# ManuelWendl/Monocular_Visual_Odometry_VA4MR

Hardware: AMD Instinct MI355X
Metric: frames/s + ATE vs ref, KITTI seq00 1241x376 @ 1/2/4/8 MI355X (higher is better)
Workload: dtype mixed(u8,i32,f32,f64)

## Files before the change

monocular_visual_odometry_va4mr_amd/csrc/vo_pyr.hip:

```cpp
#include "vo_dev.h"

namespace {


#define PT_W 128
#define PT_H 16
#ifndef PYR0_TH
#define PYR0_TH 32
#endif
#define PV_W (PT_W + 8)
#define PV_H (PT_H + 2)
#define PS_H (2 * PV_H + 3)
#define PS_W ((2 * PV_W + 3 + 8 + 3) / 4 * 4)

struct PyrLevelArgs {
    const uint8_t* src;
    int64_t sstride;
    int sw, sh, spitch;
    int64_t soff;
    uint8_t* pyr;
    int64_t pstride;
    int16_t* der;
    int64_t dstride;
    int w, h, pitch;
    int64_t off;
    int level;
};

template <bool L0, int TH, bool FSRC>
VO_DEV void pyr_tile(const PyrLevelArgs& A, int px0, int py0)
{
    constexpr int PH = TH + 2, SH = 2 * PH + 3, RPT = TH / 8;
    __shared__ uint32_t PVw[PH * PV_W / 4];
    __shared__ int yk[PH], xc[PV_W];
    __shared__ int mm[4];
    uint8_t* PV = (uint8_t*)PVw;
    const int tid = threadIdx.x;
    const int b = blockIdx.z;
    const int pw = A.w + 2 * VO_BORDER, ph = A.h + 2 * VO_BORDER;
    if (tid < 4) mm[tid] = (tid & 1) ? -1 : 0x7fffffff;
    __syncthreads();
    if (tid < PH) {
        const int py = py0 - 1 + tid;
        const int y = (py >= 0 && py < ph) ? refl101(py - VO_BORDER, A.h) : -1;
        yk[tid] = y;
        if (y >= 0) { atomicMin(&mm[0], y); atomicMax(&mm[1], y); }
    }
    if (tid < PV_W) {
        const int px = px0 - 4 + tid;
        const int x = (px >= 0 && px < pw) ? refl101(px - VO_BORDER, A.w) : -1;
        xc[tid] = x;
        if (x >= 0) { atomicMin(&mm[2], x); atomicMax(&mm[3], x); }
    }
    __syncthreads();
    constexpr int NPV = (PH * PV_W + 255) / 256;
    if constexpr (L0) {
        const uint8_t* fr = A.src + (int64_t)b * A.sstride;
        uint32_t v[NPV];
#pragma unroll
        for (int i = 0; i < NPV; ++i) {
            const int e = tid + 256 * i;
            const int ee = min(e, PH * PV_W - 1);
            const int k = ee / PV_W, c = ee - k * PV_W;
            const int y = yk[k], x = xc[c];
            v[i] = fr[(int64_t)max(y, 0) * A.w + max(x, 0)];
            if (y < 0 || x < 0) v[i] = 0;
        }
#pragma unroll
        for (int i = 0; i < NPV; ++i) {
            const int e = tid + 256 * i;
            if (e < PH * PV_W) PV[e] = (uint8_t)v[i];
        }
    } else {
        __shared__ uint32_t SRw[SH * PS_W / 4];
        __shared__ uint2 HSw[SH * PV_W / 4];
        const uint8_t* SR = (const uint8_t*)SRw;
        const int sy0 = 2 * mm[0] - 2, sy1 = 2 * mm[1] + 2;
        const int sx0 = 2 * mm[2] - 2, sx1 = 2 * mm[3] + 2;
        const int nsr = sy1 - sy0 + 1;
        const int gx0 = sx0 + VO_BORDER;
        const int ax0 = gx0 & ~3, sh = gx0 - ax0;
        const int nwd = (sx1 + VO_BORDER - ax0) / 4 + 1;
        constexpr int NSR = (SH * (PS_W / 4) + 255) / 256;
        uint32_t v[NSR];
        if constexpr (FSRC) {
            const uint8_t* fr = A.src + (int64_t)b * A.sstride;
#pragma unroll
            for (int i = 0; i < NSR; ++i) {
                const int e = tid + 256 * i;
                const int r = e / (PS_W / 4), c = e - r * (PS_W / 4);
                const bool in = r < nsr && c < nwd;
                const uint8_t* row = fr + (int64_t)refl101(sy0 + (in ? r : 0), A.sh) * A.sw;
                const int cb = ax0 - VO_BORDER + 4 * (in ? c : 0);
                v[i] = (uint32_t)row[refl101(cb, A.sw)] | ((uint32_t)row[refl101(cb + 1, A.sw)] << 8) |
                       ((uint32_t)row[refl101(cb + 2, A.sw)] << 16) | ((uint32_t)row[refl101(cb + 3, A.sw)] << 24);
            }
        } else {
            const uint8_t* sbase = A.src + (int64_t)b * A.sstride + A.soff + ax0;
#pragma unroll
            for (int i = 0; i < NSR; ++i) {
                const int e = tid + 256 * i;
                const int r = e / (PS_W / 4), c = e - r * (PS_W / 4);
                const bool in = r < nsr && c < nwd;
                v[i] = *(const uint32_t*)(sbase + (int64_t)(sy0 + (in ? r : 0) + VO_BORDER) * A.spitch + 4 * (in ? c : 0));
            }
        }
#pragma unroll
        for (int i = 0; i < NSR; ++i) {
            const int e = tid + 256 * i;
            if (e < SH * (PS_W / 4)) SRw[e] = v[i];
        }
        __syncthreads();
        static_assert(PV_W % 4 == 0, "pyrDown column quads");
        constexpr int PQ = PV_W / 4;
        uint2* HS2 = HSw;
        for (int e = tid; e < nsr * PQ; e += 256) {
            const int r = e / PQ, cq = e - r * PQ;
            const int x0 = xc[4 * cq], x3 = xc[4 * cq + 3];
            uint32_t o[4];
            if (x0 >= 0 && x3 == x0 + 3 && xc[4 * cq + 1] == x0 + 1 && xc[4 * cq + 2] == x0 + 2) {
                const int ob = r * PS_W + sh + (2 * x0 - 2 - sx0);
                const uint32_t* wp = SRw + (ob >> 2);
                const uint32_t sa = (uint32_t)(ob & 3);
                const uint32_t W0 = wp[0], W1 = wp[1], W2 = wp[2], W3 = wp[3];
                const uint32_t T0 = __builtin_amdgcn_alignbyte(W1, W0, sa);
                const uint32_t T1 = __builtin_amdgcn_alignbyte(W2, W1, sa);
                const uint32_t T2 = __builtin_amdgcn_alignbyte(W3, W2, sa);
                constexpr uint32_t K4 = 0x04060401u;
                o[0] = __builtin_amdgcn_udot4(T0, K4, T1 & 0xffu, false);
                o[1] = __builtin_amdgcn_udot4(__builtin_amdgcn_alignbyte(T1, T0, 2), K4, (T1 >> 16) & 0xffu, false);
                o[2] = __builtin_amdgcn_udot4(T1, K4, T2 & 0xffu, false);
                o[3] = __builtin_amdgcn_udot4(__builtin_amdgcn_alignbyte(T2, T1, 2), K4, (T2 >> 16) & 0xffu, false);
            } else {
#pragma unroll
                for (int i = 0; i < 4; ++i) {
                    const int x = xc[4 * cq + i];
                    o[i] = 0;
                    if (x >= 0) {
                        const uint8_t* q = SR + r * PS_W + sh + (2 * x - 2 - sx0);
                        o[i] = q[0] + 4 * q[1] + 6 * q[2] + 4 * q[3] + q[4];
                    }
                }
            }
            HS2[r * PQ + cq] = make_uint2(o[0] | (o[1] << 16), o[2] | (o[3] << 16));
        }
        __syncthreads();
        const uint2* HSq = HSw;
        for (int e = tid; e < PH * PQ; e += 256) {
            const int k = e / PQ, cq = e - k * PQ;
            const int y = yk[k];
            uint32_t v = 0;
            if (y >= 0) {
                const uint2* q = HSq + (2 * y - 2 - sy0) * PQ + cq;
                const uint2 q0 = q[0], q1 = q[PQ], q2 = q[2 * PQ], q3 = q[3 * PQ], q4 = q[4 * PQ];
                const uint32_t ax = q0.x + 4 * q1.x + 6 * q2.x + 4 * q3.x + q4.x + 0x00800080u;
                const uint32_t ay = q0.y + 4 * q1.y + 6 * q2.y + 4 * q3.y + q4.y + 0x00800080u;
                v = __builtin_amdgcn_perm(ay, ax, 0x07050301u);
            }
            PVw[k * (PV_W / 4) + cq] = v;
        }
    }    __syncthreads();
    const int tc = tid & 31, tr = tid >> 5;
    const int px = px0 + 4 * tc;
#pragma unroll
    for (int rr = 0; rr < RPT; ++rr) {
        const int k = 1 + RPT * tr + rr;
        const int py = py0 + RPT * tr + rr;
        if (py >= ph || px >= A.pitch) continue;
        const uint32_t* rowc = PVw + (k * PV_W) / 4 + 1 + tc;
        *(uint32_t*)(A.pyr + (int64_t)b * A.pstride + A.off + (int64_t)py * A.pitch + px) = rowc[0];
        const int y = py - VO_BORDER, x0 = px - VO_BORDER;
        if (!A.der || y < 0 || y >= A.h || x0 + 3 < 0 || x0 >= A.w) continue;
        uint32_t o[4];
        const uint32_t* ru = rowc - PV_W / 4;
        const uint32_t* rl = rowc + PV_W / 4;
        const uint64_t U = ((uint64_t)ru[0] << 8) | (ru[-1] >> 24), L = ((uint64_t)rl[0] << 8) | (rl[-1] >> 24),
                       Cc = ((uint64_t)rowc[0] << 8) | (rowc[-1] >> 24);
        const uint64_t U5 = U | ((uint64_t)(ru[1] & 0xff) << 40), L5 = L | ((uint64_t)(rl[1] & 0xff) << 40),
                       C5 = Cc | ((uint64_t)(rowc[1] & 0xff) << 40);
#pragma unroll
        for (int i = 0; i < 4; ++i) {
            int dx = 0, dy = 0;
            const int x = x0 + i;
            if (x >= 0 && x < A.w) {
                const int ul = (int)((U5 >> (8 * i)) & 0xff), uc = (int)((U5 >> (8 * i + 8)) & 0xff),
                          ur = (int)((U5 >> (8 * i + 16)) & 0xff);
                const int ll = (int)((L5 >> (8 * i)) & 0xff), lc = (int)((L5 >> (8 * i + 8)) & 0xff),
                          lr = (int)((L5 >> (8 * i + 16)) & 0xff);
                const int cl = (int)((C5 >> (8 * i)) & 0xff), cr = (int)((C5 >> (8 * i + 16)) & 0xff);
                const int t0l = (ul + ll) * 3 + cl * 10;
                const int t0r = (ur + lr) * 3 + cr * 10;
                dx = t0r - t0l;
                dy = ((lr - ur) + (ll - ul)) * 3 + (lc - uc) * 10;
            }
            o[i] = (uint32_t)(uint16_t)(int16_t)dx | ((uint32_t)(uint16_t)(int16_t)dy << 16);
        }
        int16_t* dq = A.der + (int64_t)b * A.dstride + 2 * (A.off + (int64_t)py * A.pitch + px);
        *(uint4*)dq = make_uint4(o[0], o[1], o[2], o[3]);
    }
}


__global__ void __launch_bounds__(256) k_pyr01(PyrLevelArgs A0, PyrLevelArgs A1, int tx0, int ty0, int tx1)
{
    if ((int)blockIdx.y < ty0) {
        if ((int)blockIdx.x < tx0) pyr_tile<true, PYR0_TH, false>(A0, blockIdx.x * PT_W, blockIdx.y * PYR0_TH);
    } else if ((int)blockIdx.x < tx1) {
        pyr_tile<false, PT_H, true>(A1, blockIdx.x * PT_W, (blockIdx.y - ty0) * PT_H);
    }
}

#define PR_STEP 248
template <bool L0, bool RAGGED = false>
VO_DEV void pyr_rows_wave(const PyrLevelArgs& A, int R, int sx, int sy, int b)
{
    const int lane = lane_id();
    const int wo = A.w, ho = A.h;
    const int pw = wo + 2 * VO_BORDER, ph = ho + 2 * VO_BORDER;
    const int pwa = (pw + 3) & ~3;
    const int ns = (pwa + PR_STEP - 1) / PR_STEP;
    const bool lastst = sx == ns - 1;
    const int base = lastst ? max(pwa - 252, -4) : sx * PR_STEP - 4;
    const int px = base + 4 * lane;
    const int y0 = sy * R;
    if (y0 >= ho || sx >= ns) return;
    const int y1 = min(y0 + R, ho);
    const int lo = lastst ? max(pwa - PR_STEP, 0) : sx * PR_STEP;
    const int hi = lastst ? pwa : min(sx * PR_STEP + PR_STEP, pwa - PR_STEP);
    const bool wlane = lane >= 1 && lane <= 62 && px >= lo && px < hi && px < pw;
    const bool dlane = wlane && px + 3 >= VO_BORDER && px < VO_BORDER + wo;
    int fsrc[4];
#pragma unroll
    for (int j = 0; j < 4; ++j) {
        const int c = px + j;
        const int sp = (c >= 0 && c < pw) ? VO_BORDER + refl101(c - VO_BORDER, wo) : c;
        const int rel = sp - base;
        fsrc[j] = (rel >= 0 && rel < 256) ? rel : 4 * lane + j;
    }
    const bool fixcols = base < VO_BORDER || base + 256 > VO_BORDER + wo;
    auto fix = [&](uint32_t v) -> uint32_t {
        if (!fixcols) return v;
        uint32_t o = 0;
#pragma unroll
        for (int j = 0; j < 4; ++j) {
            const uint32_t t = (uint32_t)__builtin_amdgcn_ds_bpermute((fsrc[j] >> 2) << 2, (int)v);
            o |= ((t >> (8 * (fsrc[j] & 3))) & 0xffu) << (8 * j);
        }
        return o;
    };
    const __amdgpu_buffer_rsrc_t rs =
        __builtin_amdgcn_make_buffer_rsrc((void*)(A.src + (int64_t)b * A.sstride), (short)0, (int)A.sstride, 0x00020000);
    uint8_t* dst = A.pyr + (int64_t)b * A.pstride + A.off;
    auto put_row = [&](int y, uint32_t v) {
        if (!wlane) return;
        *(uint32_t*)(dst + (int64_t)(VO_BORDER + y) * A.pitch + px) = v;
        if (ho >= VO_BORDER + 2) {
            if (y >= 1 && y <= VO_BORDER) *(uint32_t*)(dst + (int64_t)(VO_BORDER - y) * A.pitch + px) = v;
            if (y >= ho - 1 - VO_BORDER && y <= ho - 2)
                *(uint32_t*)(dst + (int64_t)(VO_BORDER + 2 * ho - 2 - y) * A.pitch + px) = v;
        } else {
            for (int py = 0; py < ph; ++py) {
                if (py == VO_BORDER) py = VO_BORDER + ho;
                if (py < ph && refl101(py - VO_BORDER, ho) == y) *(uint32_t*)(dst + (int64_t)py * A.pitch + px) = v;
            }
        }
    };
    auto put_der = [&](int y, uint32_t u, uint32_t c, uint32_t l) {
        const uint32_t ul = (uint32_t)__builtin_amdgcn_update_dpp(0, (int)u, 0x138, 0xF, 0xF, false);
        const uint32_t cl = (uint32_t)__builtin_amdgcn_update_dpp(0, (int)c, 0x138, 0xF, 0xF, false);
        const uint32_t ll = (uint32_t)__builtin_amdgcn_update_dpp(0, (int)l, 0x138, 0xF, 0xF, false);
        const uint32_t ur = (uint32_t)__builtin_amdgcn_update_dpp(0, (int)u, 0x130, 0xF, 0xF, false);
        const uint32_t cr = (uint32_t)__builtin_amdgcn_update_dpp(0, (int)c, 0x130, 0xF, 0xF, false);
        const uint32_t lr = (uint32_t)__builtin_amdgcn_update_dpp(0, (int)l, 0x130, 0xF, 0xF, false);
        if (!dlane || !A.der) return;
        const uint64_t U5 = ((uint64_t)u << 8) | (ul >> 24) | ((uint64_t)(ur & 0xff) << 40);
        const uint64_t L5 = ((uint64_t)l << 8) | (ll >> 24) | ((uint64_t)(lr & 0xff) << 40);
        const uint64_t C5 = ((uint64_t)c << 8) | (cl >> 24) | ((uint64_t)(cr & 0xff) << 40);
        uint32_t o[4];
#pragma unroll
        for (int i = 0; i < 4; ++i) {
            int dx = 0, dy = 0;
            const int x = px + i - VO_BORDER;
            if (x >= 0 && x < wo) {
                const int uL = (int)((U5 >> (8 * i)) & 0xff), uc = (int)((U5 >> (8 * i + 8)) & 0xff),
                          uR = (int)((U5 >> (8 * i + 16)) & 0xff);
                const int lL = (int)((L5 >> (8 * i)) & 0xff), lc = (int)((L5 >> (8 * i + 8)) & 0xff),
                          lR = (int)((L5 >> (8 * i + 16)) & 0xff);
                const int cL = (int)((C5 >> (8 * i)) & 0xff), cR = (int)((C5 >> (8 * i + 16)) & 0xff);
                dx = ((uR + lR) * 3 + cR * 10) - ((uL + lL) * 3 + cL * 10);
                dy = ((lR - uR) + (lL - uL)) * 3 + (lc - uc) * 10;
            }
            o[i] = (uint32_t)(uint16_t)(int16_t)dx | ((uint32_t)(uint16_t)(int16_t)dy << 16);
        }
        int16_t* dq = A.der + (int64_t)b * A.dstride + 2 * (A.off + (int64_t)(VO_BORDER + y) * A.pitch + px);
        *(uint4*)dq = make_uint4(o[0], o[1], o[2], o[3]);
    };
    if constexpr (L0) {
        auto ld_dw = [&](int o) -> uint32_t {
            uint32_t v = __builtin_amdgcn_raw_buffer_load_b32(rs, o, 0, 0);
            if constexpr (RAGGED) {
                const int fbytes = (int)A.sstride;
                if (o < fbytes && o + 4 > fbytes) {
                    v = 0;
#pragma unroll
                    for (int k = 0; k < 3; ++k) v |= (uint32_t)(uint8_t)__builtin_amdgcn_raw_buffer_load_b8(rs, o + k, 0, 0) << (8 * k);
                }
            }
            return v;
        };
        auto ld_row = [&](int y, uint32_t& d0, uint32_t& d1) {
            const int ro = y * wo + base - VO_BORDER;
            const int al = (ro & ~3) + 4 * lane;
            d0 = ld_dw(al);
            d1 = ld_dw(al + 4);
        };
        auto val = [&](int y, uint32_t d0, uint32_t d1) {
            return fix(__builtin_amdgcn_alignbyte(d1, d0, (uint32_t)((y * wo + base - VO_BORDER) & 3)));
        };
        uint32_t a0, a1, c0, c1, n0, n1;
        const int yh = refl101(y0 - 1, ho);
        ld_row(yh, a0, a1);
        ld_row(y0, c0, c1);
        ld_row(y0 + 1 < y1 ? y0 + 1 : refl101(y1, ho), n0, n1);
        uint32_t vu = val(yh, a0, a1);
        uint32_t vc = val(y0, c0, c1);
        put_row(y0, vc);
        for (int y = y0; y < y1; ++y) {
            const int yn = y + 1 < y1 ? y + 1 : refl101(y1, ho);
            const uint32_t vl = val(yn, n0, n1);
            const int y2 = y + 2 < y1 ? y + 2 : refl101(y1, ho);
            if (y + 1 < y1) ld_row(y2, n0, n1);
            if (y + 1 < y1) put_row(y + 1, vl);
            put_der(y, vu, vc, vl);
            vu = vc;
            vc = vl;
        }
    } else {
        const int loff = 2 * px - VO_BORDER;
        auto ld_src = [&](int sr, uint32_t& d0, uint32_t& d1) {
            const int o = (int)A.soff + (VO_BORDER + sr) * A.spitch + loff;
            d0 = __builtin_amdgcn_raw_buffer_load_b32(rs, o, 0, 0);
            d1 = __builtin_amdgcn_raw_buffer_load_b32(rs, o + 4, 0, 0);
        };
        constexpr uint32_t K4 = 0x04060401u;
        auto hsum = [&](uint32_t D0, uint32_t D1, uint32_t& h01, uint32_t& h23) {
            const uint32_t L1 = (uint32_t)__builtin_amdgcn_update_dpp(0, (int)D1, 0x138, 0xF, 0xF, false);
            const uint32_t R0 = (uint32_t)__builtin_amdgcn_update_dpp(0, (int)D0, 0x130, 0xF, 0xF, false);
            const uint32_t o0 = __builtin_amdgcn_udot4(__builtin_amdgcn_alignbyte(D0, L1, 2), K4, (D0 >> 16) & 0xffu, false);
            const uint32_t o1 = __builtin_amdgcn_udot4(D0, K4, D1 & 0xffu, false);
            const uint32_t o2 = __builtin_amdgcn_udot4(__builtin_amdgcn_alignbyte(D1, D0, 2), K4, (D1 >> 16) & 0xffu, false);
            const uint32_t o3 = __builtin_amdgcn_udot4(D1, K4, R0 & 0xffu, false);
            h01 = o0 | (o1 << 16);
            h23 = o2 | (o3 << 16);
        };
        auto vert = [&](const uint32_t (&hx)[5], const uint32_t (&hy)[5]) {
            const uint32_t ax = hx[0] + 4 * hx[1] + 6 * hx[2] + 4 * hx[3] + hx[4] + 0x00800080u;
            const uint32_t ay = hy[0] + 4 * hy[1] + 6 * hy[2] + 4 * hy[3] + hy[4] + 0x00800080u;
            return fix(__builtin_amdgcn_perm(ay, ax, 0x07050301u));
        };
        auto direct = [&](int y) {
            uint32_t d[5][2], hx[5], hy[5];
#pragma unroll
            for (int k = 0; k < 5; ++k) ld_src(2 * y - 2 + k, d[k][0], d[k][1]);
#pragma unroll
            for (int k = 0; k < 5; ++k) hsum(d[k][0], d[k][1], hx[k], hy[k]);
            return vert(hx, hy);
        };
        uint32_t hx[5], hy[5];
        {
            uint32_t d[5][2];
#pragma unroll
            for (int k = 0; k < 5; ++k) ld_src(2 * y0 - 2 + k, d[k][0], d[k][1]);
#pragma unroll
            for (int k = 0; k < 5; ++k) hsum(d[k][0], d[k][1], hx[k], hy[k]);
        }
        uint32_t p0, p1, q0, q1;
        ld_src(2 * y0 + 3, p0, p1);
        ld_src(2 * y0 + 4, q0, q1);
        uint32_t vu = direct(refl101(y0 - 1, ho));
        uint32_t vc = vert(hx, hy);
        put_row(y0, vc);
        for (int y = y0; y < y1; ++y) {
            uint32_t vl;
            if (y + 1 < y1) {
                hx[0] = hx[2]; hy[0] = hy[2];
                hx[1] = hx[3]; hy[1] = hy[3];
                hx[2] = hx[4]; hy[2] = hy[4];
                hsum(p0, p1, hx[3], hy[3]);
                hsum(q0, q1, hx[4], hy[4]);
                ld_src(2 * y + 5, p0, p1);
                ld_src(2 * y + 6, q0, q1);
                vl = vert(hx, hy);
                put_row(y + 1, vl);
            } else {
                vl = direct(refl101(y1, ho));
            }
            put_der(y, vu, vc, vl);
            vu = vc;
            vc = vl;
        }
    }
}

template <bool L0, bool RAGGED = false>
__global__ void __launch_bounds__(64) k_pyr_rows(PyrLevelArgs A, int R)
{
    pyr_rows_wave<L0, RAGGED>(A, R, (int)blockIdx.x, (int)blockIdx.y, (int)blockIdx.z);
}

#define PYR_TAIL_MAX 6
struct PyrTailArgs {
    PyrLevelArgs a[PYR_TAIL_MAX];
    int R[PYR_TAIL_MAX];
    int n;
};
__global__ void __launch_bounds__(1024) k_pyr_tail(PyrTailArgs T)
{
    const int w = wave_id(), nw = (int)(blockDim.x >> 6);
    for (int l = 0; l < T.n; ++l) {
        const PyrLevelArgs& A = T.a[l];
        const int R = T.R[l];
        const int pwa = (A.w + 2 * VO_BORDER + 3) & ~3;
        const int ns = (pwa + PR_STEP - 1) / PR_STEP, nch = (A.h + R - 1) / R;
        for (int it = w; it < ns * nch; it += nw) pyr_rows_wave<false>(A, R, it % ns, it / ns, (int)blockIdx.x);
        __syncthreads();
    }
}

__global__ void __launch_bounds__(256) k_scharr(const uint8_t* __restrict__ pyr, int64_t pstride,
                                                int16_t* __restrict__ der, int64_t dstride,
                                                int w, int h, int pitch, int64_t off)
{
    const int b = blockIdx.z;
    const int px0 = (blockIdx.x * 64 + lane_id()) * 4;
    const int py = blockIdx.y * 4 + wave_id();
    if (px0 >= w + 2 * VO_BORDER || py >= h + 2 * VO_BORDER) return;
    const int y = py - VO_BORDER;
    const uint8_t* c = pyr + b * pstride + off + (int64_t)py * pitch;
    const uint8_t* u = c - pitch;
    const uint8_t* l = c + pitch;
    uint32_t o[4];
#pragma unroll
    for (int k = 0; k < 4; ++k) {
        const int px = px0 + k, x = px - VO_BORDER;
        int dx = 0, dy = 0;
        if (x >= 0 && x < w && y >= 0 && y < h) {
            const int t0l = (u[px - 1] + l[px - 1]) * 3 + c[px - 1] * 10;
            const int t0r = (u[px + 1] + l[px + 1]) * 3 + c[px + 1] * 10;
            const int t1l = l[px - 1] - u[px - 1], t1c = l[px] - u[px], t1r = l[px + 1] - u[px + 1];
            dx = t0r - t0l;
            dy = (t1r + t1l) * 3 + t1c * 10;
        }
        o[k] = (uint32_t)(uint16_t)(int16_t)dx | ((uint32_t)(uint16_t)(int16_t)dy << 16);
    }
    int16_t* dq = der + b * dstride + 2 * (off + (int64_t)py * pitch + px0);
    *(uint4*)dq = make_uint4(o[0], o[1], o[2], o[3]);
}

}

static bool pyr_level_args(const vo_dims* d, const vo_state* s, int cur, int l, const uint8_t* frames,
                           int64_t frame_stride, PyrLevelArgs* A)
{
    if (l == 0) {
        A->src = frames; A->sstride = frame_stride; A->sw = A->sh = A->spitch = 0; A->soff = 0;
    } else {
        A->src = s->pyr[cur]; A->sstride = d->pyr_stride;
        A->sw = d->lvl_w[l - 1]; A->sh = d->lvl_h[l - 1]; A->spitch = d->lvl_pitch[l - 1]; A->soff = d->lvl_off[l - 1];
    }
    A->pyr = s->pyr[cur]; A->pstride = d->pyr_stride;
    A->der = s->der[cur]; A->dstride = d->der_stride;
    A->w = d->lvl_w[l]; A->h = d->lvl_h[l]; A->pitch = d->lvl_pitch[l]; A->off = d->lvl_off[l];
    A->level = l;
    return A->pitch % 64 == 0 && A->pitch >= A->w + 2 * VO_BORDER;
}

extern "C" int vo_pyr_build(const vo_dims* d, const vo_state* s, int cur, const uint8_t* frames,
                            int64_t frame_stride, vo_stream_t stream)
{
    if (!d || !s || !frames || cur < 0 || cur > 1 || d->nlev < 1) return VO_EARG;
    static const int p01_env = vo_env_int("VO_PYR01", -1);
    const bool fuse01 = d->nlev >= 2 && (p01_env >= 0 ? p01_env == 1 : d->B <= 8);
    if (fuse01) {
        PyrLevelArgs A0, A1;
        if (!pyr_level_args(d, s, cur, 0, frames, frame_stride, &A0)) return VO_EARG;
        if (!pyr_level_args(d, s, cur, 1, frames, frame_stride, &A1)) return VO_EARG;
        A1.src = frames; A1.sstride = frame_stride; A1.spitch = 0; A1.soff = 0;
        const int pw0 = A0.w + 2 * VO_BORDER, ph0 = A0.h + 2 * VO_BORDER;
        const int pw1 = A1.w + 2 * VO_BORDER, ph1 = A1.h + 2 * VO_BORDER;
        const int tx0 = (pw0 + PT_W - 1) / PT_W, ty0 = (ph0 + PYR0_TH - 1) / PYR0_TH;
        const int tx1 = (pw1 + PT_W - 1) / PT_W, ty1 = (ph1 + PT_H - 1) / PT_H;
        dim3 g(tx0 > tx1 ? tx0 : tx1, ty0 + ty1, d->B);
        hipLaunchKernelGGL(k_pyr01, g, dim3(256), 0, VO_STREAM(stream), A0, A1, tx0, ty0, tx1);
    }
    static const int tail_env = vo_env_int("VO_PYR_TAIL", -1);
    const int ltail = 2;
    const bool tail = d->nlev > ltail && d->nlev - ltail <= PYR_TAIL_MAX &&
                      (tail_env >= 0 ? tail_env == 1 : d->B > 8 && d->B <= 64);
    PyrTailArgs T;
    T.n = tail ? d->nlev - ltail : 0;
    for (int i = 0; i < T.n; ++i) {
        PyrLevelArgs& A = T.a[i];
        if (!pyr_level_args(d, s, cur, ltail + i, frames, frame_stride, &A)) return VO_EARG;
        const int pwa = (A.w + 2 * VO_BORDER + 3) & ~3, ns = (pwa + PR_STEP - 1) / PR_STEP;
        const int want = ns >= 16 ? 1 : 16 / ns;
        const int R = (A.h + want - 1) / want;
        T.R[i] = R < 2 ? 2 : R;
    }
    const int lend = tail ? ltail : d->nlev;
    for (int l = fuse01 ? 2 : 0; l < lend; ++l) {
        PyrLevelArgs A;
        if (!pyr_level_args(d, s, cur, l, frames, frame_stride, &A)) return VO_EARG;
        const int pw = A.w + 2 * VO_BORDER;
        const int ns = ((pw + 3) / 4 * 4 + PR_STEP - 1) / PR_STEP;
        int R = 16;
        while (R > 4 && (int64_t)ns * ((A.h + R - 1) / R) * d->B < 8192) R >>= 1;
        dim3 g(ns, (A.h + R - 1) / R, d->B);
        if (l == 0 && (frame_stride & 3)) hipLaunchKernelGGL((k_pyr_rows<true, true>), g, dim3(64), 0, VO_STREAM(stream), A, R);
        else if (l == 0) hipLaunchKernelGGL(k_pyr_rows<true>, g, dim3(64), 0, VO_STREAM(stream), A, R);
        else hipLaunchKernelGGL(k_pyr_rows<false>, g, dim3(64), 0, VO_STREAM(stream), A, R);
    }
    if (tail) hipLaunchKernelGGL(k_pyr_tail, dim3(d->B), dim3(1024), 0, VO_STREAM(stream), T);
    return hip_ok() ? VO_OK : VO_EHIP;
}

extern "C" int vo_pyr_deriv(const vo_dims* d, const vo_state* s, int which, vo_stream_t stream)
{
    if (!d || !s || which < 0 || which > 1) return VO_EARG;
    for (int l = 0; l < d->nlev; ++l) {
        const int pw = d->lvl_w[l] + 2 * VO_BORDER, ph = d->lvl_h[l] + 2 * VO_BORDER;
        dim3 g((pw + 4 * 64 - 1) / (4 * 64), (ph + 3) / 4, d->B);
        hipLaunchKernelGGL(k_scharr, g, dim3(256), 0, VO_STREAM(stream), s->pyr[which], d->pyr_stride, s->der[which],
                           d->der_stride, d->lvl_w[l], d->lvl_h[l], d->lvl_pitch[l], d->lvl_off[l]);
    }
    return hip_ok() ? VO_OK : VO_EHIP;
}
```

Before: 86860.

## Vectorize pyramid Scharr derivative with packed 16-bit math and buffer stores

Rewrites the per-row derivative computation in the pyramid row kernel to use packed 16-bit vector arithmetic on unpacked byte pairs, with DPP lane shifts and alignbyte instead of per-pixel 64-bit shifting. Adds a specialized inner-row loop, split on whether column fixup is needed, that removes reflection branches and uses incremental offsets. Stores go through buffer resources, L1+ levels load with 64-bit buffer loads, and a waves-per-EU occupancy hint plus a readfirstlane are added. Together these cut ALU and branch overhead in the pyramid/derivative stage. The cost is more code paths and a border-masking scheme that must keep matching the previous output.

Result: no change. 87650 (median of 6 runs) (+0.9%).

```diff
diff --git a/monocular_visual_odometry_va4mr_amd/csrc/vo_pyr.hip b/monocular_visual_odometry_va4mr_amd/csrc/vo_pyr.hip
--- a/monocular_visual_odometry_va4mr_amd/csrc/vo_pyr.hip
+++ b/monocular_visual_odometry_va4mr_amd/csrc/vo_pyr.hip
@@ -1,3 +1,5 @@
+#include <type_traits>
+
 #include "vo_dev.h"
 
 namespace {
@@ -211,6 +213,21 @@
 }
 
 #define PR_STEP 248
+typedef unsigned short pr_u16x2 __attribute__((ext_vector_type(2)));
+typedef short pr_i16x2 __attribute__((ext_vector_type(2)));
+typedef uint32_t pr_u32x2 __attribute__((ext_vector_type(2)));
+typedef uint32_t pr_u32x4 __attribute__((ext_vector_type(4)));
+struct PrRow { uint32_t lo, hi; };
+VO_DEV PrRow pr_unpack(uint32_t v)
+{
+    return PrRow{__builtin_amdgcn_perm(0u, v, 0x0c010c00u), __builtin_amdgcn_perm(0u, v, 0x0c030c02u)};
+}
+VO_DEV uint32_t pr_shr(uint32_t v) { return (uint32_t)__builtin_amdgcn_mov_dpp((int)v, 0x138, 0xF, 0xF, true); }
+VO_DEV uint32_t pr_shl(uint32_t v) { return (uint32_t)__builtin_amdgcn_mov_dpp((int)v, 0x130, 0xF, 0xF, true); }
+VO_DEV pr_u16x2 pr_u16(uint32_t v) { return __builtin_bit_cast(pr_u16x2, v); }
+VO_DEV pr_i16x2 pr_i16(uint32_t v) { return __builtin_bit_cast(pr_i16x2, v); }
+VO_DEV uint32_t pr_u32(pr_u16x2 v) { return __builtin_bit_cast(uint32_t, v); }
+VO_DEV uint32_t pr_u32(pr_i16x2 v) { return __builtin_bit_cast(uint32_t, v); }
 template <bool L0, bool RAGGED = false>
 VO_DEV void pyr_rows_wave(const PyrLevelArgs& A, int R, int sx, int sy, int b)
 {
@@ -228,18 +245,26 @@
     const int lo = lastst ? max(pwa - PR_STEP, 0) : sx * PR_STEP;
     const int hi = lastst ? pwa : min(sx * PR_STEP + PR_STEP, pwa - PR_STEP);
     const bool wlane = lane >= 1 && lane <= 62 && px >= lo && px < hi && px < pw;
-    const bool dlane = wlane && px + 3 >= VO_BORDER && px < VO_BORDER + wo;
+    const bool dlane = wlane && A.der && px + 3 >= VO_BORDER && px < VO_BORDER + wo;
+    const bool fixcols = base < VO_BORDER || base + 256 > VO_BORDER + wo;
     int fsrc[4];
+    uint32_t dmask[4];
+    bool part = false;
 #pragma unroll
     for (int j = 0; j < 4; ++j) {
         const int c = px + j;
-        const int sp = (c >= 0 && c < pw) ? VO_BORDER + refl101(c - VO_BORDER, wo) : c;
-        const int rel = sp - base;
-        fsrc[j] = (rel >= 0 && rel < 256) ? rel : 4 * lane + j;
-    }
-    const bool fixcols = base < VO_BORDER || base + 256 > VO_BORDER + wo;
-    auto fix = [&](uint32_t v) -> uint32_t {
-        if (!fixcols) return v;
+        fsrc[j] = 4 * lane + j;
+        if (fixcols) {
+            const int sp = (c >= 0 && c < pw) ? VO_BORDER + refl101(c - VO_BORDER, wo) : c;
+            const int rel = sp - base;
+            if (rel >= 0 && rel < 256) fsrc[j] = rel;
+        }
+        const bool in = c >= VO_BORDER && c < VO_BORDER + wo;
+        dmask[j] = in ? 0xffffffffu : 0u;
+        part |= !in;
+    }
+    const bool partcols = __ballot(dlane && part) != 0;
+    auto fixv = [&](uint32_t v) -> uint32_t {
         uint32_t o = 0;
 #pragma unroll
         for (int j = 0; j < 4; ++j) {
@@ -248,52 +273,56 @@
         }
         return o;
     };
+    auto fix = [&](uint32_t v) -> uint32_t { return fixcols ? fixv(v) : v; };
     const __amdgpu_buffer_rsrc_t rs =
         __builtin_amdgcn_make_buffer_rsrc((void*)(A.src + (int64_t)b * A.sstride), (short)0, (int)A.sstride, 0x00020000);
-    uint8_t* dst = A.pyr + (int64_t)b * A.pstride + A.off;
+    const __amdgpu_buffer_rsrc_t rp =
+        __builtin_amdgcn_make_buffer_rsrc((void*)(A.pyr + (int64_t)b * A.pstride), (short)0, (int)A.pstride, 0x00020000);
+    const __amdgpu_buffer_rsrc_t rd =
+        __builtin_amdgcn_make_buffer_rsrc((void*)(A.der + (int64_t)b * A.dstride), (short)0, (int)(2 * A.dstride), 0x00020000);
+    auto row_off = [&](int py) { return (int)A.off + py * A.pitch; };
+    auto st_row = [&](int ro, uint32_t v) { __builtin_amdgcn_raw_buffer_store_b32(v, rp, px, ro, 0); };
     auto put_row = [&](int y, uint32_t v) {
         if (!wlane) return;
-        *(uint32_t*)(dst + (int64_t)(VO_BORDER + y) * A.pitch + px) = v;
+        st_row(row_off(VO_BORDER + y), v);
         if (ho >= VO_BORDER + 2) {
-            if (y >= 1 && y <= VO_BORDER) *(uint32_t*)(dst + (int64_t)(VO_BORDER - y) * A.pitch + px) = v;
-            if (y >= ho - 1 - VO_BORDER && y <= ho - 2)
-                *(uint32_t*)(dst + (int64_t)(VO_BORDER + 2 * ho - 2 - y) * A.pitch + px) = v;
+            if (y >= 1 && y <= VO_BORDER) st_row(row_off(VO_BORDER - y), v);
+            if (y >= ho - 1 - VO_BORDER && y <= ho - 2) st_row(row_off(VO_BORDER + 2 * ho - 2 - y), v);
         } else {
             for (int py = 0; py < ph; ++py) {
                 if (py == VO_BORDER) py = VO_BORDER + ho;
-                if (py < ph && refl101(py - VO_BORDER, ho) == y) *(uint32_t*)(dst + (int64_t)py * A.pitch + px) = v;
+                if (py < ph && refl101(py - VO_BORDER, ho) == y) st_row(row_off(py), v);
             }
         }
     };
-    auto put_der = [&](int y, uint32_t u, uint32_t c, uint32_t l) {
-        const uint32_t ul = (uint32_t)__builtin_amdgcn_update_dpp(0, (int)u, 0x138, 0xF, 0xF, false);
-        const uint32_t cl = (uint32_t)__builtin_amdgcn_update_dpp(0, (int)c, 0x138, 0xF, 0xF, false);
-        const uint32_t ll = (uint32_t)__builtin_amdgcn_update_dpp(0, (int)l, 0x138, 0xF, 0xF, false);
-        const uint32_t ur = (uint32_t)__builtin_amdgcn_update_dpp(0, (int)u, 0x130, 0xF, 0xF, false);
-        const uint32_t cr = (uint32_t)__builtin_amdgcn_update_dpp(0, (int)c, 0x130, 0xF, 0xF, false);
-        const uint32_t lr = (uint32_t)__builtin_amdgcn_update_dpp(0, (int)l, 0x130, 0xF, 0xF, false);
-        if (!dlane || !A.der) return;
-        const uint64_t U5 = ((uint64_t)u << 8) | (ul >> 24) | ((uint64_t)(ur & 0xff) << 40);
-        const uint64_t L5 = ((uint64_t)l << 8) | (ll >> 24) | ((uint64_t)(lr & 0xff) << 40);
-        const uint64_t C5 = ((uint64_t)c << 8) | (cl >> 24) | ((uint64_t)(cr & 0xff) << 40);
-        uint32_t o[4];
-#pragma unroll
-        for (int i = 0; i < 4; ++i) {
-            int dx = 0, dy = 0;
-            const int x = px + i - VO_BORDER;
-            if (x >= 0 && x < wo) {
-                const int uL = (int)((U5 >> (8 * i)) & 0xff), uc = (int)((U5 >> (8 * i + 8)) & 0xff),
-                          uR = (int)((U5 >> (8 * i + 16)) & 0xff);
-                const int lL = (int)((L5 >> (8 * i)) & 0xff), lc = (int)((L5 >> (8 * i + 8)) & 0xff),
-                          lR = (int)((L5 >> (8 * i + 16)) & 0xff);
-                const int cL = (int)((C5 >> (8 * i)) & 0xff), cR = (int)((C5 >> (8 * i + 16)) & 0xff);
-                dx = ((uR + lR) * 3 + cR * 10) - ((uL + lL) * 3 + cL * 10);
-                dy = ((lR - uR) + (lL - uL)) * 3 + (lc - uc) * 10;
-            }
-            o[i] = (uint32_t)(uint16_t)(int16_t)dx | ((uint32_t)(uint16_t)(int16_t)dy << 16);
-        }
-        int16_t* dq = A.der + (int64_t)b * A.dstride + 2 * (A.off + (int64_t)(VO_BORDER + y) * A.pitch + px);
-        *(uint4*)dq = make_uint4(o[0], o[1], o[2], o[3]);
+    const bool inner = ho >= VO_BORDER + 2 && y0 >= VO_BORDER && y1 < ho - 1 - VO_BORDER;
+    auto put_der = [&](int ro, const PrRow& u, const PrRow& c, const PrRow& l, bool pm) {
+        const uint32_t Tl = pr_u32((pr_u16(u.lo) + pr_u16(l.lo)) * (unsigned short)3 + pr_u16(c.lo) * (unsigned short)10);
+        const uint32_t Th = pr_u32((pr_u16(u.hi) + pr_u16(l.hi)) * (unsigned short)3 + pr_u16(c.hi) * (unsigned short)10);
+        const uint32_t Vl = pr_u32(pr_i16(l.lo) - pr_i16(u.lo));
+        const uint32_t Vh = pr_u32(pr_i16(l.hi) - pr_i16(u.hi));
+        const uint32_t TL = pr_shr(Th);
+        const uint32_t VL = pr_shr(Vh);
+        const uint32_t TR = pr_shl(Tl);
+        const uint32_t VR = pr_shl(Vl);
+        if (!dlane) return;
+        const uint32_t Tm = __builtin_amdgcn_alignbyte(Tl, TL, 2), Tc = __builtin_amdgcn_alignbyte(Th, Tl, 2),
+                       Tp = __builtin_amdgcn_alignbyte(TR, Th, 2);
+        const uint32_t Vm = __builtin_amdgcn_alignbyte(Vl, VL, 2), Vc = __builtin_amdgcn_alignbyte(Vh, Vl, 2),
+                       Vp = __builtin_amdgcn_alignbyte(VR, Vh, 2);
+        const uint32_t dxl = pr_u32(pr_i16(Tc) - pr_i16(Tm)), dxh = pr_u32(pr_i16(Tp) - pr_i16(Tc));
+        const uint32_t dyl = pr_u32((pr_i16(Vm) + pr_i16(Vc)) * (short)3 + pr_i16(Vl) * (short)10);
+        const uint32_t dyh = pr_u32((pr_i16(Vc) + pr_i16(Vp)) * (short)3 + pr_i16(Vh) * (short)10);
+        pr_u32x4 o;
+        o[0] = __builtin_amdgcn_perm(dyl, dxl, 0x05040100u);
+        o[1] = __builtin_amdgcn_perm(dyl, dxl, 0x07060302u);
+        o[2] = __builtin_amdgcn_perm(dyh, dxh, 0x05040100u);
+        o[3] = __builtin_amdgcn_perm(dyh, dxh, 0x07060302u);
+        if (pm) {
+#pragma unroll
+            for (int j = 0; j < 4; ++j) o[j] &= dmask[j];
+        }
+        __builtin_amdgcn_raw_buffer_store_b128(o, rd, 4 * px, 4 * ro, 0);
     };
     if constexpr (L0) {
         auto ld_dw = [&](int o) -> uint32_t {
@@ -317,35 +346,70 @@
         auto val = [&](int y, uint32_t d0, uint32_t d1) {
             return fix(__builtin_amdgcn_alignbyte(d1, d0, (uint32_t)((y * wo + base - VO_BORDER) & 3)));
         };
-        uint32_t a0, a1, c0, c1, n0, n1;
-        const int yh = refl101(y0 - 1, ho);
-        ld_row(yh, a0, a1);
-        ld_row(y0, c0, c1);
-        ld_row(y0 + 1 < y1 ? y0 + 1 : refl101(y1, ho), n0, n1);
-        uint32_t vu = val(yh, a0, a1);
-        uint32_t vc = val(y0, c0, c1);
-        put_row(y0, vc);
-        for (int y = y0; y < y1; ++y) {
-            const int yn = y + 1 < y1 ? y + 1 : refl101(y1, ho);
-            const uint32_t vl = val(yn, n0, n1);
-            const int y2 = y + 2 < y1 ? y + 2 : refl101(y1, ho);
-            if (y + 1 < y1) ld_row(y2, n0, n1);
-            if (y + 1 < y1) put_row(y + 1, vl);
-            put_der(y, vu, vc, vl);
-            vu = vc;
-            vc = vl;
+        uint32_t n0 = 0, n1 = 0;
+        PrRow U, C, L;
+        {
+            uint32_t a0, a1, c0, c1;
+            const int yh = refl101(y0 - 1, ho);
+            ld_row(yh, a0, a1);
+            ld_row(y0, c0, c1);
+            if (y0 + 1 < ho) ld_row(y0 + 1, n0, n1);
+            U = pr_unpack(val(yh, a0, a1));
+            const uint32_t vc = val(y0, c0, c1);
+            put_row(y0, vc);
+            C = pr_unpack(vc);
+        }
+        int y = y0;
+        if (inner) {
+            auto run = [&](auto FX) {
+                int fo = (y0 + 2) * wo + base - VO_BORDER;
+                int sp = row_off(VO_BORDER + y0 + 1), sd = row_off(VO_BORDER + y0);
+                for (; y < y1 - 1; ++y) {
+                    uint32_t vl = __builtin_amdgcn_alignbyte(n1, n0, (uint32_t)((fo - wo) & 3));
+                    if (decltype(FX)::value) vl = fixv(vl);
+                    const int al = (fo & ~3) + 4 * lane;
+                    n0 = __builtin_amdgcn_raw_buffer_load_b32(rs, al, 0, 0);
+                    n1 = __builtin_amdgcn_raw_buffer_load_b32(rs, al + 4, 0, 0);
+                    if (wlane) st_row(sp, vl);
+                    L = pr_unpack(vl);
+                    put_der(sd, U, C, L, decltype(FX)::value && partcols);
+                    U = C;
+                    C = L;
+                    fo += wo;
+                    sp += A.pitch;
+                    sd += A.pitch;
+                }
+            };
+            if (fixcols) run(std::true_type{});
+            else run(std::false_type{});
+        }
+        for (; y < y1; ++y) {
+            if (y + 1 < ho) {
+                const uint32_t vl = val(y + 1, n0, n1);
+                if (y + 1 < y1) {
+                    if (y + 2 < ho) ld_row(y + 2, n0, n1);
+                    put_row(y + 1, vl);
+                }
+                L = pr_unpack(vl);
+            } else {
+                L = U;
+            }
+            put_der(row_off(VO_BORDER + y), U, C, L, partcols);
+            U = C;
+            C = L;
         }
     } else {
         const int loff = 2 * px - VO_BORDER;
-        auto ld_src = [&](int sr, uint32_t& d0, uint32_t& d1) {
-            const int o = (int)A.soff + (VO_BORDER + sr) * A.spitch + loff;
-            d0 = __builtin_amdgcn_raw_buffer_load_b32(rs, o, 0, 0);
-            d1 = __builtin_amdgcn_raw_buffer_load_b32(rs, o + 4, 0, 0);
-        };
+        auto ld8 = [&](int so, uint32_t& d0, uint32_t& d1) {
+            const pr_u32x2 d = __builtin_amdgcn_raw_buffer_load_b64(rs, so + loff, 0, 0);
+            d0 = d[0];
+            d1 = d[1];
+        };
+        auto ld_src = [&](int sr, uint32_t& d0, uint32_t& d1) { ld8((int)A.soff + (VO_BORDER + sr) * A.spitch, d0, d1); };
         constexpr uint32_t K4 = 0x04060401u;
         auto hsum = [&](uint32_t D0, uint32_t D1, uint32_t& h01, uint32_t& h23) {
-            const uint32_t L1 = (uint32_t)__builtin_amdgcn_update_dpp(0, (int)D1, 0x138, 0xF, 0xF, false);
-            const uint32_t R0 = (uint32_t)__builtin_amdgcn_update_dpp(0, (int)D0, 0x130, 0xF, 0xF, false);
+            const uint32_t L1 = pr_shr(D1);
+            const uint32_t R0 = pr_shl(D0);
             const uint32_t o0 = __builtin_amdgcn_udot4(__builtin_amdgcn_alignbyte(D0, L1, 2), K4, (D0 >> 16) & 0xffu, false);
             const uint32_t o1 = __builtin_amdgcn_udot4(D0, K4, D1 & 0xffu, false);
             const uint32_t o2 = __builtin_amdgcn_udot4(__builtin_amdgcn_alignbyte(D1, D0, 2), K4, (D1 >> 16) & 0xffu, false);
@@ -353,11 +417,12 @@
             h01 = o0 | (o1 << 16);
             h23 = o2 | (o3 << 16);
         };
-        auto vert = [&](const uint32_t (&hx)[5], const uint32_t (&hy)[5]) {
+        auto vraw = [&](const uint32_t* hx, const uint32_t* hy) {
             const uint32_t ax = hx[0] + 4 * hx[1] + 6 * hx[2] + 4 * hx[3] + hx[4] + 0x00800080u;
             const uint32_t ay = hy[0] + 4 * hy[1] + 6 * hy[2] + 4 * hy[3] + hy[4] + 0x00800080u;
-            return fix(__builtin_amdgcn_perm(ay, ax, 0x07050301u));
-        };
+            return __builtin_amdgcn_perm(ay, ax, 0x07050301u);
+        };
+        auto vert = [&](const uint32_t* hx, const uint32_t* hy) { return fix(vraw(hx, hy)); };
         auto direct = [&](int y) {
             uint32_t d[5][2], hx[5], hy[5];
 #pragma unroll
@@ -367,43 +432,87 @@
             return vert(hx, hy);
         };
         uint32_t hx[5], hy[5];
+        uint32_t p0, p1, q0, q1;
+        PrRow U, C, L;
+        if (y0 >= 1) {
+            uint32_t d[7][2], gx[7], gy[7];
+#pragma unroll
+            for (int k = 0; k < 7; ++k) ld_src(2 * y0 - 4 + k, d[k][0], d[k][1]);
+#pragma unroll
+            for (int k = 0; k < 7; ++k) hsum(d[k][0], d[k][1], gx[k], gy[k]);
+            ld_src(2 * y0 + 3, p0, p1);
+            ld_src(2 * y0 + 4, q0, q1);
+            U = pr_unpack(vert(gx, gy));
+#pragma unroll
+            for (int k = 0; k < 5; ++k) { hx[k] = gx[k + 2]; hy[k] = gy[k + 2]; }
+        } else {
+            uint32_t d[5][2];
+#pragma unroll
+            for (int k = 0; k < 5; ++k) ld_src(2 * y0 - 2 + k, d[k][0], d[k][1]);
+#pragma unroll
+            for (int k = 0; k < 5; ++k) hsum(d[k][0], d[k][1], hx[k], hy[k]);
+            ld_src(2 * y0 + 3, p0, p1);
+            ld_src(2 * y0 + 4, q0, q1);
+            U = pr_unpack(direct(refl101(-1, ho)));
+        }
         {
-            uint32_t d[5][2];
-#pragma unroll
-            for (int k = 0; k < 5; ++k) ld_src(2 * y0 - 2 + k, d[k][0], d[k][1]);
-#pragma unroll
-            for (int k = 0; k < 5; ++k) hsum(d[k][0], d[k][1], hx[k], hy[k]);
-        }
-        uint32_t p0, p1, q0, q1;
-        ld_src(2 * y0 + 3, p0, p1);
-        ld_src(2 * y0 + 4, q0, q1);
-        uint32_t vu = direct(refl101(y0 - 1, ho));
-        uint32_t vc = vert(hx, hy);
-        put_row(y0, vc);
-        for (int y = y0; y < y1; ++y) {
-            uint32_t vl;
-            if (y + 1 < y1) {
-                hx[0] = hx[2]; hy[0] = hy[2];
-                hx[1] = hx[3]; hy[1] = hy[3];
-                hx[2] = hx[4]; hy[2] = hy[4];
-                hsum(p0, p1, hx[3], hy[3]);
-                hsum(q0, q1, hx[4], hy[4]);
-                ld_src(2 * y + 5, p0, p1);
-                ld_src(2 * y + 6, q0, q1);
-                vl = vert(hx, hy);
-                put_row(y + 1, vl);
+            const uint32_t vc = vert(hx, hy);
+            put_row(y0, vc);
+            C = pr_unpack(vc);
+        }
+        auto advance = [&]() {
+            hx[0] = hx[2]; hy[0] = hy[2];
+            hx[1] = hx[3]; hy[1] = hy[3];
+            hx[2] = hx[4]; hy[2] = hy[4];
+            hsum(p0, p1, hx[3], hy[3]);
+            hsum(q0, q1, hx[4], hy[4]);
+        };
+        int y = y0;
+        if (inner) {
+            auto run = [&](auto FX) {
+                int so = (int)A.soff + (VO_BORDER + 2 * y0 + 5) * A.spitch;
+                int sp = row_off(VO_BORDER + y0 + 1), sd = row_off(VO_BORDER + y0);
+                for (; y < y1 - 1; ++y) {
+                    advance();
+                    ld8(so, p0, p1);
+                    ld8(so + A.spitch, q0, q1);
+                    uint32_t vl = vraw(hx, hy);
+                    if (decltype(FX)::value) vl = fixv(vl);
+                    if (wlane) st_row(sp, vl);
+                    L = pr_unpack(vl);
+                    put_der(sd, U, C, L, decltype(FX)::value && partcols);
+                    U = C;
+                    C = L;
+                    so += 2 * A.spitch;
+                    sp += A.pitch;
+                    sd += A.pitch;
+                }
+            };
+            if (fixcols) run(std::true_type{});
+            else run(std::false_type{});
+        }
+        for (; y < y1; ++y) {
+            if (y + 1 < ho) {
+                advance();
+                if (y + 1 < y1) {
+                    ld_src(2 * y + 5, p0, p1);
+                    ld_src(2 * y + 6, q0, q1);
+                }
+                const uint32_t vl = vert(hx, hy);
+                if (y + 1 < y1) put_row(y + 1, vl);
+                L = pr_unpack(vl);
             } else {
-                vl = direct(refl101(y1, ho));
-            }
-            put_der(y, vu, vc, vl);
-            vu = vc;
-            vc = vl;
+                L = U;
+            }
+            put_der(row_off(VO_BORDER + y), U, C, L, partcols);
+            U = C;
+            C = L;
         }
     }
 }
 
 template <bool L0, bool RAGGED = false>
-__global__ void __launch_bounds__(64) k_pyr_rows(PyrLevelArgs A, int R)
+__global__ void __launch_bounds__(64) __attribute__((amdgpu_waves_per_eu(8))) k_pyr_rows(PyrLevelArgs A, int R)
 {
     pyr_rows_wave<L0, RAGGED>(A, R, (int)blockIdx.x, (int)blockIdx.y, (int)blockIdx.z);
 }
@@ -416,7 +525,7 @@
 };
 __global__ void __launch_bounds__(1024) k_pyr_tail(PyrTailArgs T)
 {
-    const int w = wave_id(), nw = (int)(blockDim.x >> 6);
+    const int w = __builtin_amdgcn_readfirstlane(wave_id()), nw = (int)(blockDim.x >> 6);
     for (int l = 0; l < T.n; ++l) {
         const PyrLevelArgs& A = T.a[l];
         const int R = T.R[l];
```
